# EDM-Research/Real-time-Neural-Rendering-of-LiDAR-Point-Clouds

Hardware: AMD Instinct MI355X
Metric: Mpoints/sec projected + frames/sec at 1920x1080 (higher is better)
Workload: dtype f32

## Files before the change

### real-time-neural-rendering-of-lidar-point-clouds_amd/csrc/rtr_api.hip

```cpp
#include <hip/hip_runtime.h>

#include <algorithm>
#include <cmath>
#include <cstdarg>
#include <cstdio>
#include <cstring>
#include <functional>
#include <string>
#include <vector>

#include "rtr_host.h"
#include "rtr_extract_index.h"

constexpr int kSplitCooldown = 8;

static thread_local std::string g_create_err;

int fail(rtr_ctx *c, int code, const char *fmt, ...) {
    char buf[512];
    va_list ap;
    va_start(ap, fmt);
    vsnprintf(buf, sizeof buf, fmt, ap);
    va_end(ap);
    if (c) c->err = buf; else g_create_err = buf;
// ... 74 lines not shown
    t.cap = 0;
}

int alloc_target(rtr_ctx *c, rtr_ctx::Target &t, int count) {
    free_target(t);
    const size_t npix = (size_t)c->W * c->H, n = (size_t)count * npix;
    const size_t nparts = (size_t)((c->W + 31) / 32) * ((c->H + 31) / 32);
    hipError_t e = rtr::dev_malloc(&t.depth, n * 4);
    if (e == hipSuccess) e = rtr::dev_malloc(&t.img, (n * 3 + 15) & ~(size_t)15);
    if (e == hipSuccess) e = rtr::dev_malloc(&t.tensor, n * 5 * sizeof(uint16_t));
    if (e == hipSuccess) e = rtr::dev_malloc(&t.acc, npix * 16);
    if (e == hipSuccess) e = rtr::dev_malloc(&t.mask, npix);
    if (e == hipSuccess) e = rtr::dev_malloc(&t.part_min, nparts * 4);
    if (e == hipSuccess) e = rtr::dev_malloc(&t.part_max, nparts * 4);
    if (e != hipSuccess) {
        free_target(t);
        return fail(c, RTR_ERR_HIP, "hipMalloc of the frame buffers (%d x %dx%d) failed: %s", count, c->W, c->H,
                    hipGetErrorString(e));
    }
    t.cap = count;
    return RTR_OK;
}

void free_frame(rtr_ctx *c) {
    c->list_valid = false;
    c->split_cooldown = kSplitCooldown;
    free_host_out(c);
    p2p_release(c);
    dfree(c->pp_ids);
    for (auto *t : {&c->frame, &c->views}) {
        free_target(*t);
        for (auto &f : t->fs) {
            dfree(f.store.ext0); dfree(f.store.meta);
            f.nst = f.ntiles = 0;
            f.consts = rtr::StoreConsts{};
        }
    }
    c->W = c->H = 0;
    c->jr.views.count = 0;
}

void reset_pool_sizing(rtr_ctx::Target &t) {
    t.pool_worst = false;
    t.entries_max = 0;
    if (t.entries_host) *t.entries_host = 0u;
}

void free_lists(rtr_ctx *c) {
    if (c->p2p.open || c->p2p.red) p2p_release(c);
    for (auto *t : {&c->frame, &c->views})
        for (auto &f : t->fs) {
            dfree(f.dyn);
            f.dyn_cap = 0;
            f.pool_n = 0;
        }
    c->list_valid = false;
    c->split_cooldown = kSplitCooldown;
    reset_pool_sizing(c->frame);
// ... 180 lines not shown
    rtr_ctx *c; int k; hipStream_t s; hipEvent_t a = nullptr, b = nullptr;
    bool in_dispatch;
    Timed(rtr_ctx *c_, int k_, hipStream_t s_ = nullptr, bool in_dispatch_ = false)
        : c(c_), k(k_), s(s_ ? s_ : c_->stream), in_dispatch(in_dispatch_) {
        if (!c->timing) return;
        if (c->timing >= 2 && k != RTR_K_MIN_DEPTH && k != RTR_K_ACCUMULATE) return;
        if (c->timing == 3 && (c->timing_tick++ & 3u) != 0u) return;
        if (c->timing == 4 && (c->timing_tick++ & 1u) != 0u) return;
        if (c->pool.empty()) {
            (void)hipEventCreate(&a); (void)hipEventCreate(&b);
        } else {
            a = c->pool.back().first; b = c->pool.back().second; c->pool.pop_back();
        }
        if (!in_dispatch) (void)hipEventRecord(a, s);
    }
    ~Timed() {
        if (!a) return;
        if (!in_dispatch) (void)hipEventRecord(b, s);
        c->pending.push_back({a, b, k});
    }
};

hipError_t sync_streams(rtr_ctx *c) {
    if (c->front) {
        hipError_t e = hipStreamSynchronize(c->front);
        if (e != hipSuccess) return e;
    }
    return hipStreamSynchronize(c->stream);
}

#ifndef RTR_DISPATCH_EVENTS
#define RTR_DISPATCH_EVENTS 3
#endif

hipEvent_t consumed_in_dispatch(rtr_ctx *c) {
    if (!(RTR_DISPATCH_EVENTS & 1) || !c->front || !c->frame_overlapped) return nullptr;
    return c->F().consumed;
}

void mark_consumed(rtr_ctx *c, bool in_dispatch = false) {
    if (!c->front || !(c->ov.mode == 1 || c->frame_overlapped)) return;
    auto &f = c->F();
    if (in_dispatch || hipEventRecord(f.consumed, c->stream) == hipSuccess) f.consumed_valid = true;
}

int collect_timing(rtr_ctx *c) {
    if (c->pending.empty()) return RTR_OK;
    HIP_TRY(c, sync_streams(c));
    for (auto &s : c->pending) {
        float ms = 0.f;
        if (hipEventElapsedTime(&ms, s.a, s.b) == hipSuccess) {
            c->total_ms[s.k] += ms;
            c->launches[s.k] += 1;
        }
        c->pool.emplace_back(s.a, s.b);
    }
    c->pending.clear();
    return RTR_OK;
}

int check_frame(rtr_ctx *c) {
    NEED(c, c->W > 0 && c->H > 0, "rtr_set_resolution has not been called");
    return RTR_OK;
}

int check_prefilter(rtr_ctx *c) {
// ... 13 lines not shown
    t.lv_levels = 0;
    for (int i = 1, w = c->W / 2, h = c->H / 2; i <= L; ++i, w /= 2, h /= 2) {
        const hipError_t e = rtr::dev_malloc(&t.lv[i], sizeof(float) * (size_t)w * h);
        if (e != hipSuccess) {
            for (auto &l : t.lv) dfree(l);
            return fail(c, RTR_ERR_HIP, "allocating pyramid level %d (%dx%d) failed: %s", i, w, h, hipGetErrorString(e));
        }
    }
    t.lv_levels = L;
    return RTR_OK;
}

int ensure_pyramid(rtr_ctx *c) {
    if (int rc = check_prefilter(c)) return rc;
    return ensure_levels(c, c->frame);
}

rtr::FilterLevels levels_of(const rtr_ctx *c, const rtr_ctx::Target &t, int k) {
    rtr::FilterLevels L{};
    L.levels = t.lv_levels;
    L.lv[0] = reinterpret_cast<float *>(t.depth + (size_t)k * c->W * c->H);
    L.w[0] = c->W; L.h[0] = c->H;
    for (int i = 1; i <= L.levels; ++i) L.lv[i] = t.lv[i], L.w[i] = L.w[i - 1] / 2, L.h[i] = L.h[i - 1] / 2;
    return L;
}

rtr::TilePyr tile_pyr(const rtr_ctx *c, const rtr_ctx::Target &t, int k, bool enable) {
    rtr::TilePyr pyr{};
    pyr.enable = enable ? 1 : 0;
    if (enable) {
        pyr.L = levels_of(c, t, k);
        pyr.n_eff_rows = (uint32_t)((c->H >> 4) << 4);
        pyr.part_min = t.part_min;
        pyr.part_max = t.part_max;
    }
    return pyr;
}

}

void free_select(rtr_ctx *c) {
    if (!c->sel) return;
    (void)sync_streams(c);
    dfree(c->sel); dfree(c->sel_stats);
}

// ... 116 lines not shown
    if (c->vtab.copied) (void)hipEventDestroy(c->vtab.copied);
    if (c->copy_stream) (void)hipStreamDestroy(c->copy_stream);
    if (c->pp_done) (void)hipEventDestroy(c->pp_done);
    if (c->own_stream) (void)hipStreamDestroy(c->own_stream);
    delete c;
    return RTR_OK;
}

const char *rtr_last_error(const rtr_ctx *c) { return c ? c->err.c_str() : g_create_err.c_str(); }

int rtr_set_params(rtr_ctx *c, const rtr_params *p) {
    if (!c) return RTR_ERR_INVALID;
    c->ov.other_call();
    NEED(c, p != nullptr, "params is NULL");
    NEED(c, p->levels >= 1 && p->levels <= 8, "levels must be in 1..8");
    c->prm = *p;
    c->list_valid = false;
    return RTR_OK;
}

static void overlap_teardown(rtr_ctx *c) {
    if (c->masked_tail && c->stream == c->masked_tail) c->stream = c->own_stream;
    if (c->front) (void)hipStreamDestroy(c->front);
    if (c->masked_tail) (void)hipStreamDestroy(c->masked_tail);
    c->front = c->masked_tail = nullptr;
    for (auto &f : c->frame.fs) {
        if (f.binned) (void)hipEventDestroy(f.binned);
        if (f.consumed) (void)hipEventDestroy(f.consumed);
        f.binned = f.consumed = nullptr;
        f.consumed_valid = false;
    }
    if (c->joined) (void)hipEventDestroy(c->joined);
    c->joined = nullptr;
}

static hipError_t overlap_streams(rtr_ctx *c) {
    if (c->front) return hipSuccess;
    hipError_t e = hipSuccess;
    if (c->ov.mode == 1 && c->opt_tail_cus > 0) {
        uint32_t tail[8] = {0}, head[8] = {0};
        for (int i = 0; i < 256; ++i) {
            int a = i % 8, b = (i / 8) % 4, x = i / 32;
            bool is_tail = b * 8 + (a + x) % 8 < c->opt_tail_cus;
            (is_tail ? tail : head)[i / 32] |= 1u << (i % 32);
        }
        e = hipExtStreamCreateWithCUMask(&c->front, 8, head);
        if (e == hipSuccess) e = hipExtStreamCreateWithCUMask(&c->masked_tail, 8, tail);
        if (e == hipSuccess && c->stream == c->own_stream) c->stream = c->masked_tail;
    } else if (c->opt_front_priority) {
        int least = 0, greatest = 0;
        e = hipDeviceGetStreamPriorityRange(&least, &greatest);
        if (e == hipSuccess) e = hipStreamCreateWithPriority(&c->front, hipStreamNonBlocking, c->opt_front_priority == 1 ? least : greatest);
    } else {
        e = hipStreamCreateWithFlags(&c->front, hipStreamNonBlocking);
    }
    for (int k = 0; k < 2 && e == hipSuccess; ++k) {
        auto &f = c->frame.fs[k];
        e = hipEventCreateWithFlags(&f.binned, hipEventDisableTiming);
        if (e == hipSuccess) e = hipEventCreateWithFlags(&f.consumed, hipEventDisableTiming);
        f.consumed_valid = false;
    }
    if (e == hipSuccess) e = hipEventCreateWithFlags(&c->joined, hipEventDisableTiming);
    if (e != hipSuccess) overlap_teardown(c);
    return e;
}

static int set_overlap(rtr_ctx *c, int value) {
    NEED(c, value >= -1 && value <= 1, "overlap: -1 (automatic), 0 or 1");
    if (value == c->ov.mode && value != 0) return RTR_OK;
    if (value == 1 && c->p2p.open) return fail(c, RTR_ERR_INVALID, "option overlap cannot be switched on while the peer-to-peer exchange is open (rtr_p2p_close first)");
    DevGuard g(c->device);
    HIP_TRY(c, sync_streams(c));
    (void)collect_timing(c);
    if (value == 1 && c->opt_tail_cus > 0) {
        int ncu = 0;
        HIP_TRY(c, hipDeviceGetAttribute(&ncu, hipDeviceAttributeMultiprocessorCount, c->device));
        if (ncu != 256) return fail(c, RTR_ERR_UNSUPPORTED, "tail_cus needs the 256-CU / 8-XCD part (device has %d CUs)", ncu);
    }
    overlap_teardown(c);
    c->ov.set_mode(value);
    if (value == 0) {
        auto &o = c->frame.fs[c->frame.cur ^ 1];
        if (!(c->frame.cur == 1 && (c->p2p.open || c->p2p.red))) {
            dfree(o.dyn); dfree(o.store.ext0); dfree(o.store.meta);
            o.dyn_cap = o.pool_n = 0;
            o.nst = o.ntiles = 0;
            o.consts = rtr::StoreConsts{};
            o.parity = 0;
            o.lean_pending = false;
        }
        return RTR_OK;
    }
    if (value == 1) {
        const hipError_t e = overlap_streams(c);
        if (e != hipSuccess) {
            c->ov.set_mode(0);
            return fail(c, RTR_ERR_HIP, "option overlap: creating the front stream failed: %s", hipGetErrorString(e));
        }
    }
    return RTR_OK;
}

static bool overlap_ready(rtr_ctx *c) {
    if (overlap_streams(c) != hipSuccess) {
        (void)hipGetLastError();
        return false;
    }
    if (c->ov.mode == 1) return true;
    auto &o = c->frame.fs[c->frame.cur ^ 1];
    const std::string err = c->err;
    if (ensure_pool(c, c->frame, o, 0) != RTR_OK || ensure_store(c, c->frame, o, 0, c->front) != RTR_OK) {
        (void)hipGetLastError();
        c->err = err;
        dfree(o.dyn); dfree(o.store.ext0); dfree(o.store.meta);
        o.dyn_cap = o.pool_n = 0;
        o.nst = o.ntiles = 0;
        o.consts = rtr::StoreConsts{};
        return false;
    }
    return true;
}

static int pack_cloud(rtr_ctx *c);

int rtr_set_option(rtr_ctx *c, const char *key, int value) {
    if (!c) return RTR_ERR_INVALID;
    if (key && !strcmp(key, "debug_alloc_fail")) {
        NEED(c, value >= 0, "debug_alloc_fail must be >= 0 (0: off)");
        rtr::alloc_rule().arm(value);
        return RTR_OK;
    }
    c->ov.other_call();
    NEED(c, key != nullptr, "key is NULL");
    if (!strcmp(key, "mode")) {
        NEED(c, value == 0 || value == 1, "mode must be 0 or 1");
        c->opt_mode = value;
        c->list_valid = false;
        return RTR_OK;
    }
    if (!strcmp(key, "point_grid")) {
// ... 178 lines not shown
    else if (!strcmp(key, "nearest_chunks_skipped")) *value = c->nearest_chunks[0];
    else if (!strcmp(key, "nearest_chunks_decoded")) *value = c->nearest_chunks[1];
    else if (!strcmp(key, "nearest_k_given_us")) *value = c->nearest_k_us[0];
    else if (!strcmp(key, "nearest_k_sweep_us")) *value = c->nearest_k_us[1];
    else if (!strcmp(key, "nearest_k_pair_tests_k")) *value = c->nearest_k_tests_k;
    else if (!strcmp(key, "nearest_k_chunks_skipped")) *value = c->nearest_k_chunks[0];
    else if (!strcmp(key, "nearest_k_chunks_decoded")) *value = c->nearest_k_chunks[1];
    else if (!strcmp(key, "nearest_k_cascades_k")) *value = c->nearest_k_cascades_k;
    else if (!strcmp(key, "clusters_keys_us")) *value = c->clusters_us[0];
    else if (!strcmp(key, "clusters_sort_us")) *value = c->clusters_us[1];
    else if (!strcmp(key, "clusters_label_us")) *value = c->clusters_us[2];
    else if (!strcmp(key, "clusters_pair_tests_k")) *value = c->clusters_tests_k;
    else if (!strcmp(key, "plane_sample_us")) *value = c->plane_us[0];
    else if (!strcmp(key, "plane_count_us")) *value = c->plane_us[1];
    else if (!strcmp(key, "point_keep")) *value = c->keep_up ? 1 : 0;
    else if (!strcmp(key, "order_ratio_ppm")) *value = (int)(c->order_ratio * 1e6f);
    else if (!strcmp(key, "cull")) *value = c->opt_cull;
    else if (!strcmp(key, "point_ids")) *value = c->opt_point_ids;
    else if (!strcmp(key, "lane_test")) *value = c->opt_lane_test;
    else if (!strcmp(key, "chunk_test")) *value = c->opt_chunk_test;
    else if (!strcmp(key, "phases")) *value = c->opt_phases;
    else if (!strcmp(key, "overlap")) *value = c->ov.mode;
    else if (!strcmp(key, "overlap_active")) *value = c->ov.active ? 1 : 0;
    else if (!strcmp(key, "front_priority")) *value = c->opt_front_priority;
    else if (!strcmp(key, "lean")) *value = c->opt_lean;
    else if (!strcmp(key, "lean_identity")) *value = c->opt_lean_identity;
    else if (!strcmp(key, "lean_early")) *value = c->opt_lean_early;
    else if (!strcmp(key, "p2p_open")) *value = c->p2p.open ? 1 : 0;
    else if (!strcmp(key, "keep_soa")) *value = c->opt_keep_soa;
    else if (!strcmp(key, "pool_worst_case")) *value = c->opt_pool_worst;
    else if (!strcmp(key, "views")) *value = c->jr.views.count;
    else if (!strcmp(key, "resident_millibytes_per_point")) {
        const uint64_t nchunks = ((c->cap / 4) + 63) / 64;
        uint64_t b = (c->x ? 12 * c->cap : 0) + (c->rgba ? 4 * c->cap : 0) + nchunks * 28 +
                     (c->pk_hdr ? c->pk_bytes + (c->pk_units_cap - c->pk_units) * 32 + 64 : 0) +
                     (c->perm ? 4 * c->cap : 0) + (c->keep_up ? (c->n + 31) / 32 * 4 + nchunks * 33 + 4 : 0) +
                     (c->sel ? std::max<uint64_t>((c->n + 255) / 256, 1) * 32 + 32 : 0);
        const uint64_t npix = (uint64_t)c->W * c->H;
        for (const auto *t : {&c->frame, &c->views}) {
            for (const auto &f : t->fs) {
                b += f.dyn ? f.dyn_cap * 8 : 0;
                b += f.store.ext0 ? ((uint64_t)f.nst * rtr::kS0 + 16) * 8 + rtr::ts_meta_words(f.nst, f.ntiles) * 4 : 0;
            }
            b += t->cap ? npix * (16 + 1 + (uint64_t)t->cap * (4 + 3 + 10)) : 0;
        }
        *value = c->n ? (int)((b * 1000) / c->n > 0x7FFFFFFFull ? 0x7FFFFFFF : (b * 1000) / c->n) : 0;
// ... 1192 lines not shown
    c->W = W; c->H = H;
    if (int rc = alloc_target(c, c->frame, 1)) {
        c->W = c->H = 0;
        return rc;
    }
    return RTR_OK;
}


int rtr_clear(rtr_ctx *c) {
    if (!c) return RTR_ERR_INVALID;
    c->ov.other_call();
    if (int rc = check_frame(c)) return rc;
    DevGuard g(c->device);
    { Timed t(c, RTR_K_CLEAR); rtr::launch_clear(c->stream, c->frame.depth, c->frame.acc, (size_t)c->W * c->H); }
    return launch_check(c, "clear");
}

static bool use_tiles(const rtr_ctx *c) {
    return c->opt_mode == 1 && !c->force_atomic && rtr::tile_count(c->W, c->H) <= 4096;
}

static int bin_points(rtr_ctx *c, const float P[16], bool overlapped, bool clear_split, bool no_split = false,
                      bool lean = false) {
    c->list_valid = false;
    c->last_lean = false;
    c->p2p.occ_current = false;
    c->p2p.occ_from_scan = false;
    hipStream_t s1 = c->stream;
    if (overlapped) {
        if (!c->ov.active) {
            HIP_TRY(c, hipEventRecord(c->joined, c->stream));
            HIP_TRY(c, hipStreamWaitEvent(c->front, c->joined, 0));
        }
        c->frame.cur ^= 1;
        s1 = c->front;
        if (c->F().consumed_valid) HIP_TRY(c, hipStreamWaitEvent(c->front, c->F().consumed, 0));
    }
    if (int rc = ensure_pool(c, c->frame, c->F(), 0)) return rc;
    if (int rc = ensure_store(c, c->frame, c->F(), 0, s1)) return rc;
    auto &t = c->F().store;
    if (c->F().lean_pending && !lean) rtr::launch_lean_fold(s1, c->W, c->H, t, c->F().parity);
    c->F().lean_pending = lean;
    const bool heavy_seen = c->split_cooldown > 0 || __atomic_load_n(c->split_host, __ATOMIC_RELAXED) != 0u;
    t.fill_shift = c->opt_fill_shift >= 0 ? c->opt_fill_shift : (heavy_seen ? 4 : 1);
    if (int rc = next_seq(c, c->F(), s1)) return rc;
    bool binned_in_dispatch = false;
    {
        Timed tm(c, RTR_K_MIN_DEPTH, s1, true);
        binned_in_dispatch = (RTR_DISPATCH_EVENTS & 2) && overlapped && !tm.a && (c->n > 0 || !lean);
        rtr::launch_project_bin(s1, cloud_of(c), make_proj(P), c->W, c->H, t, c->opt_cull ? c->bounds : nullptr,
                                t1_flags(c, clear_split, no_split, lean), c->opt_phases, c->opt_xp, tm.a,
                                binned_in_dispatch ? c->F().binned : tm.b);
        c->p2p.occ_from_scan = c->p2p.open;
    }
    if (overlapped) {
        if (!binned_in_dispatch) HIP_TRY(c, hipEventRecord(c->F().binned, c->front));
        HIP_TRY(c, hipStreamWaitEvent(c->stream, c->F().binned, 0));
    }
    memcpy(c->list_P, P, sizeof c->list_P);
    c->list_valid = true;
    return RTR_OK;
}

int rtr_min_depth_pass(rtr_ctx *c, const float P[16]) {
    if (!c) return RTR_ERR_INVALID;
    c->ov.other_call();
    NEED(c, P != nullptr, "P is NULL");
    if (int rc = check_frame(c)) return rc;
    DevGuard g(c->device);
    c->list_valid = false;
    c->jr.frame.count = 0;
    if (use_tiles(c)) {
        c->frame.pool_worst = true;
        if (int rc = bin_points(c, P, false, c->p2p.whole_frame)) return rc;
        Timed t(c, RTR_K_TILE);
        rtr::launch_tile(c->stream, 1, c->W, c->H, c->F().store, c->prm.depth_window, c->frame.depth, c->frame.acc, c->frame.img,
                         (c->p2p.whole_frame ? 6 : 0) | (c->F().parity << 4), nullptr);
        mark_consumed(c);
// ... 43 lines not shown
int rtr_resolve(rtr_ctx *c) {
    if (!c) return RTR_ERR_INVALID;
    c->ov.other_call();
    if (int rc = check_frame(c)) return rc;
    DevGuard g(c->device);
    { Timed t(c, RTR_K_RESOLVE); rtr::launch_resolve(c->stream, c->frame.acc, c->frame.img, (size_t)c->W * c->H); }
    return launch_check(c, "resolve");
}

int rtr_resolve_range(rtr_ctx *c, const void *acc_dev, uint64_t first_pixel, uint64_t count) {
    if (!c) return RTR_ERR_INVALID;
    c->ov.other_call();
    if (int rc = check_frame(c)) return rc;
    const uint64_t npix = (uint64_t)c->W * c->H;
    NEED(c, first_pixel % 4 == 0 && first_pixel + count <= npix, "bad pixel range (first must be a multiple of 4)");
    if (count == 0) return RTR_OK;
    DevGuard g(c->device);
    const uint32_t *src = acc_dev ? static_cast<const uint32_t *>(acc_dev) : c->frame.acc + first_pixel * 4;
    { Timed t(c, RTR_K_RESOLVE); rtr::launch_resolve(c->stream, src, c->frame.img + first_pixel * 3, (size_t)count); }
    return launch_check(c, "resolve_range");
}

static int filter_impl(rtr_ctx *c, int pyramid_parts, const rtr::Sliced *img_slices = nullptr,
                       const uint32_t *depth_src = nullptr) {
    if (int rc = check_frame(c)) return rc;
    DevGuard g(c->device);
    if (int rc = ensure_pyramid(c)) return rc;
    {
        Timed t(c, RTR_K_FILTER);
        rtr::launch_filter(c->stream, levels_of(c, c->frame, 0), c->frame.depth, c->frame.img, c->frame.mask, c->frame.tensor, c->frame.minmax, c->frame.part_min, c->frame.part_max,
                           c->W, c->H, c->prm.filter_strength, c->prm.gradient_threshold, pyramid_parts, img_slices,
                           depth_src);
    }
    return launch_check(c, "filter");
}

int rtr_filter(rtr_ctx *c) {
    if (!c) return RTR_ERR_INVALID;
    c->ov.other_call();
    return filter_impl(c, 0);
}


int rtr_render(rtr_ctx *c, const float P[16], int with_filter) {
    if (!c) return RTR_ERR_INVALID;
    NEED(c, P != nullptr, "P is NULL");
    if (int rc = check_frame(c)) return rc;
    c->jr.pass.behind = false;
    if (with_filter) {
        DevGuard g(c->device);
        if (int rc = ensure_pyramid(c)) return rc;
    }
    int rc;
    bool fused = false;
    if (use_tiles(c)) {
        DevGuard g(c->device);
        bool overlapped = c->ov.frame(!c->p2p.open && (c->ov.mode == 1 || !c->p2p.red), with_filter != 0, c->W, c->H, c->cloud_seq);
        if (overlapped && !c->ov.active && !overlap_ready(c)) {
            c->ov.resources_failed();
            overlapped = false;
        }
        c->frame_overlapped = overlapped;
        bool split_launch = c->opt_heavy > 0;
        if (split_launch) {
            if (__atomic_load_n(c->split_host, __ATOMIC_RELAXED) != 0u) c->split_cooldown = kSplitCooldown;
            split_launch = c->split_cooldown > 0;
            if (c->split_cooldown > 0) --c->split_cooldown;
        }
        const bool lean = c->opt_lean && !split_launch && !c->p2p.open;
        if ((rc = bin_points(c, P, overlapped, !overlapped, !split_launch, lean))) {
            c->frame_overlapped = false;
            c->ov.other_call();
            return rc;
        }
        if (lean) {
            c->F().parity ^= 1;
            c->last_lean = true;
        }
        if (overlapped && split_launch) rtr::launch_reset_split(c->stream, c->W, c->H, c->F().store, c->frame.depth, c->frame.acc);
        fused = with_filter && c->prm.levels == 4;
        const rtr::TilePyr pyr = tile_pyr(c, c->frame, 0, fused);
        const hipEvent_t consumed = consumed_in_dispatch(c);
        {
            Timed t(c, RTR_K_TILE);
            rtr::launch_tile(c->stream, 0, c->W, c->H, c->F().store, c->prm.depth_window, c->frame.depth, c->frame.acc, c->frame.img,
                             c->opt_keep_accum | (lean ? lean_bits(c, c->frame) : 0) | (c->F().parity << 4), fused ? &pyr : nullptr,
                             nullptr, split_launch ? nullptr : consumed);
            if (lean) c->list_valid = false;
            if (split_launch)
                rtr::launch_tile(c->stream, 3, c->W, c->H, c->F().store, c->prm.depth_window, c->frame.depth, c->frame.acc, c->frame.img,
                                 c->opt_keep_accum, fused ? &pyr : nullptr, nullptr, consumed);
        }
        mark_consumed(c, consumed != nullptr);
        c->frame_overlapped = false;
        c->ov.frame_done(overlapped);
        if ((rc = launch_check(c, "tile frame"))) return rc;
        auto &rec = c->jr.frame;
        memcpy(rec.P, P, sizeof(float) * 16);
        rec.filter = with_filter;
        rec.count = 1;
        rec.clip = c->clip;
    } else {
        (void)c->ov.frame(false, false, c->W, c->H, c->cloud_seq);
        c->ov.frame_done(false);
        c->force_atomic = true;
        rc = rtr_clear(c);
        if (!rc) rc = rtr_min_depth_pass(c, P);
        if (!rc) rc = rtr_accumulate_pass(c, P);
        if (!rc) rc = rtr_resolve(c);
        c->force_atomic = false;
        if (rc) return rc;
    }
    if (with_filter) return filter_impl(c, fused ? rtr::tile_count(c->W, c->H) : 0);
    return RTR_OK;
}

static int frame_to_host(rtr_ctx *c, const float P[16], uint8_t *host_img, float *host_depth, int with_filter) {
    if (!c) return RTR_ERR_INVALID;
    if (!host_img && !host_depth) return fail(c, RTR_ERR_NO_OUTPUT, "both outputs are NULL (project_cloud.cu:270-273)");
    c->ov.other_call();
    if (int rc = rtr_render(c, P, with_filter)) return rc;
    DevGuard g(c->device);
    const size_t npix = (size_t)c->W * c->H;
    const Copy copies[2] = {{host_depth, c->frame.depth, npix * 4}, {host_img, c->frame.img, npix * 3}};
    HIP_TRY(c, queue_copies(c, copies, 2));
    HIP_TRY(c, sync_streams(c));
    rtr_ctx::Journal::Frames own;
    memcpy(own.P, P, sizeof(float) * 16);
    own.count = 1;
    own.filter = with_filter;
    own.clip = c->clip;
    return repair(c, c->frame, false, copies, 2, &own);
}

int rtr_project(rtr_ctx *c, const float P[16], uint8_t *host_img, float *host_depth) {
    return frame_to_host(c, P, host_img, host_depth, 0);
// ... 654 lines not shown
```

### real-time-neural-rendering-of-lidar-point-clouds_amd/csrc/rtr_host.h

```cpp
#pragma once
#include <hip/hip_runtime.h>

#include <string>
#include <utility>
#include <vector>

#include "../../include/rtr.h"
#include "rtr_alloc.h"
#include "rtr_kernels.h"
#include "rtr_overlap_policy.h"

struct rtr_ctx {
    int device = 0;
    hipStream_t own_stream = nullptr;
    hipStream_t stream = nullptr;
    rtr_params prm{};
    std::string err;

    float *x = nullptr, *y = nullptr, *z = nullptr;
    uint32_t *rgba = nullptr;
    float *bounds = nullptr;
    float *spread = nullptr;
    float absmax[3] = {0.f, 0.f, 0.f};
    int opt_lane_test = 1;
// ... 4 lines not shown
    int opt_lean_identity = 1;
    int opt_lean_early = -1;
    bool last_lean = false;
    uint64_t n = 0, cap = 0;
    uint4 *pk_hdr = nullptr;
    uint32_t *pk_planes = nullptr, *pk_planes_b = nullptr;
    uint64_t pk_bytes = 0;
    uint64_t pk_units = 0, pk_units_cap = 0;
    uint64_t pk_hdr_chunks = 0;
    int opt_pack = 1;

    int W = 0, H = 0;
    rtr::Clip clip{};

    struct FrontSet {
        rtr::TileStore store{};
        uint64_t pool_n = 0;
        int nst = 0, ntiles = 0;
        rtr::StoreConsts consts{};
        uint64_t *dyn = nullptr;
        uint64_t dyn_cap = 0;
        hipEvent_t binned = nullptr, consumed = nullptr;
        bool consumed_valid = false;
        int parity = 0;
        bool lean_pending = false;
    };

    struct Target {
        int cap = 0;
        uint32_t *depth = nullptr, *acc = nullptr, *part_min = nullptr, *part_max = nullptr;
        uint8_t *img = nullptr, *mask = nullptr;
        uint16_t *tensor = nullptr;
        uint32_t *minmax = nullptr;
        float *lv[9] = {nullptr};
        int lv_levels = 0;
        FrontSet fs[RTR_MAX_VIEWS];
        int cur = 0;
        uint32_t *err_host = nullptr, *err_dev = nullptr;
        uint32_t *entries_host = nullptr, *entries_dev = nullptr;
        uint64_t entries_max = 0;
        bool pool_worst = false;
    } frame, views;
    FrontSet &F() { return frame.fs[frame.cur]; }
    rtr::OverlapPolicy ov;
    bool frame_overlapped = false;
    int opt_front_priority = 0;
    int opt_tail_cus = 0;
    hipStream_t front = nullptr;
    hipStream_t masked_tail = nullptr;
    hipEvent_t joined = nullptr;
    bool list_valid = false;
    float list_P[12] = {0};
    int opt_mode = 1;
    int opt_keep_accum = 0;
    bool force_atomic = false;
    int opt_heavy = 32768;
    int opt_slice = 16384;
    int opt_p2p_timeout_ms = 2000;
    int opt_fill_shift = -1;
    int opt_debug_dyn_cap = -1;
    int opt_debug_extract_window = -1;
    uint32_t debug_store_stamp = 0;
    int opt_debug_p2p_barrier = -1;
    uint32_t *split_host = nullptr, *split_dev = nullptr;
    int split_cooldown = 0;
    int opt_xp = 0;
    int opt_phases = 0;
    int opt_probe = 0;
    int opt_cull = 0;
    int opt_auto_reorder = 2;
    bool reordered = false;
// ... 172 lines not shown
```

### real-time-neural-rendering-of-lidar-point-clouds_amd/csrc/rtr_kernels.h

```cpp
#pragma once
#include <hip/hip_runtime.h>
#include <stdint.h>

#include "rtr_barrier_rule.h"
#include "rtr_chunk_box.h"
#include "rtr_stamp_rule.h"

namespace rtr {

struct Proj {
    float m[12];
};

constexpr uint32_t kPackMaxBits = 25;
struct PackedXyz {
    const uint4 *hdr;
    const uint32_t *planes;
    const uint32_t *planes_b;
};
constexpr uint64_t pack_b_dwords(uint64_t units) { return (units * 2 + 256 + 16 + 15) & ~15ull; }
constexpr uint64_t pack_total_dwords(uint64_t units) { return pack_b_dwords(units) + units * 6 + 16; }

struct Cloud {
    const float *x, *y, *z;
// ... 138 lines not shown
size_t view_tab_bytes();
hipError_t launch_project_bin_views(hipStream_t s, const Cloud &c, const Proj *P, const TileStore *S, int count, int W, int H,
                              void *tab_host, void *tab_dev, int flags, int phases, hipEvent_t ev_start = nullptr,
                              hipEvent_t ev_stop = nullptr);
void launch_chunk_bounds(hipStream_t s, const Cloud &c, float *bounds, float *spread);
void pack_measure(hipStream_t s, const Cloud &c, uint4 *hdr, uint32_t *chunk_planes, uint64_t *total_planes,
                  uint64_t first_unit = 0);
void pack_write(hipStream_t s, const Cloud &c, const uint4 *hdr, uint32_t *planes, uint32_t *planes_b);
void pack_verify(hipStream_t s, const Cloud &c, const uint4 *hdr, const uint32_t *planes, const uint32_t *planes_b, uint64_t *mismatches);
void unpack_to_soa(hipStream_t s, const PackedXyz &pk, uint64_t n, float *x, float *y, float *z);
int reorder_morton(hipStream_t s, float *x, float *y, float *z, uint32_t *rgba, uint64_t n, uint32_t *perm = nullptr);
size_t order_quality_scratch_bytes();
int order_quality(hipStream_t s, const float *bounds, uint64_t n, float *ratio, float absmax[3], void *scratch = nullptr);
void launch_reset_split(hipStream_t s, int W, int H, const TileStore &S, uint32_t *depth, uint32_t *acc);
void launch_tile(hipStream_t s, int mode, int W, int H, const TileStore &S, float window, uint32_t *depth,
                 uint32_t *acc, uint8_t *img, int write_acc, const TilePyr *pyr, const Sliced *depth_slices = nullptr,
                 hipEvent_t ev_stop = nullptr);
void launch_lean_fold(hipStream_t s, int W, int H, const TileStore &S, int parity);
void launch_stream_probe(hipStream_t s, const Cloud &c, const Proj &P, int W, int H, uint32_t *sink, int variant);
void launch_resolve(hipStream_t s, const uint32_t *acc, uint8_t *img, size_t npix);
void launch_filter(hipStream_t s, const FilterLevels &L, uint32_t *depth_bits, uint8_t *img, uint8_t *mask,
                   uint16_t *tensor, uint32_t *minmax, uint32_t *part_min, uint32_t *part_max, int W, int H,
                   float strength, float thr, int pyramid_parts, const Sliced *img_slices = nullptr,
                   const uint32_t *depth_src = nullptr);
void launch_p2p_sync(hipStream_t s, uint32_t *my_flags, const PeerSet &peer_flags, int rank, int world, uint32_t seq,
                     uint32_t *status, unsigned long long timeout_ticks);
void launch_p2p_sync_gather(hipStream_t s, uint32_t *my_flags, const PeerSet &peer_flags, int rank, int world, uint32_t seq,
                            uint32_t *status, unsigned long long timeout_ticks, const PeerSet &occ, uint32_t *occ_all);
constexpr int kP2POccBytes = 512;
void launch_p2p_collect(hipStream_t s, int W, int H, const OwnedTab *tab, const uint32_t *occ_all, int world, int rank,
                        uint32_t *depth, uint8_t *img, const TilePyr *pyr);
void launch_p2p_occupancy(hipStream_t s, const uint32_t *tile_cnt, int W, int H, uint32_t *occ);
void launch_p2p_depth_reduce(hipStream_t s, const PeerSet &depth, const PeerSet &occ, uint32_t *red, size_t first,
                             size_t count, int world, int W, int H);
void launch_p2p_gather(hipStream_t s, const PeerSet &src, void *dst, size_t chunk_bytes, size_t nbytes,
                       int skip_owner);
void launch_p2p_acc_resolve(hipStream_t s, const PeerSet &acc, const PeerSet &occ, uint8_t *img, size_t first,
                            size_t count, int world, int W, int H);
void launch_generate(hipStream_t s, int scene, uint64_t seed, uint64_t first, uint64_t count, uint64_t total,
                     float *x, float *y, float *z, uint32_t *rgba);
void launch_aos_to_soa(hipStream_t s, const uint8_t *xyz, size_t xyz_stride, const uint8_t *rgb, size_t rgb_stride,
                       uint64_t count, float *x, float *y, float *z, uint32_t *rgba);
void launch_soa_to_aos(hipStream_t s, const float *x, const float *y, const float *z, const uint32_t *rgba,
                       uint64_t count, float *xyzw, uint8_t *rgba_out);
void launch_copy_to_host(hipStream_t s, const void *a, void *ha, size_t bytes_a, const void *b, void *hb, size_t bytes_b);
void launch_pad_nan(hipStream_t s, float *x, float *y, float *z, uint32_t *rgba, uint64_t n, uint64_t n_pad);
void launch_point_pass(hipStream_t s, const Cloud &c, const Proj &P, int W, int H, const uint32_t *depth, float window,
// ... 108 lines not shown
```

### real-time-neural-rendering-of-lidar-point-clouds_amd/csrc/rtr_kernels.hip

```cpp
#include "rtr_device.h"
#include "rtr_lane_test.h"
#include "rtr_remove_index.h"
#include "rtr_extract_index.h"

#include <hip/hip_ext.h>
#include <hip/hip_fp16.h>

#include <type_traits>

namespace rtr {

__global__ __launch_bounds__(kBlock) void k_clear(uint4 *__restrict__ depth4, uint4 *__restrict__ acc4,
                                                  size_t n_depth4, size_t n_acc4, uint32_t *depth, size_t npix) {
    size_t i = (size_t)blockIdx.x * kBlock + threadIdx.x;
    size_t stride = (size_t)gridDim.x * kBlock;
    const uint4 e = make_uint4(RTR_EMPTY, RTR_EMPTY, RTR_EMPTY, RTR_EMPTY);
    const uint4 z = make_uint4(0, 0, 0, 0);
    for (size_t j = i; j < n_acc4; j += stride) acc4[j] = z;
    for (size_t j = i; j < n_depth4; j += stride) depth4[j] = e;
    for (size_t j = n_depth4 * 4 + i; j < npix; j += stride) depth[j] = RTR_EMPTY;
}

void launch_clear(hipStream_t s, uint32_t *depth, uint32_t *acc, size_t npix) {
    size_t n_acc4 = npix, n_depth4 = npix / 4;
// ... 3017 lines not shown
        const int gx = ox + q % SX, gy = oy + q / SX;
        if (gx < 0 || gx >= hw || gy < 0 || gy >= hh) continue;
        if (!keep_px(lo, hi[q], gx, gy, strength, thr)) hi[q] = bilerp(lo, gx, gy);
    }
}

#ifdef RTR_EXPERIMENT
__device__ unsigned long long g_fstamp[2][8];
#define RTR_FSTAMP(k) do { if (threadIdx.x == 0 && (blockIdx.x == 5 || blockIdx.x == 1900)) g_fstamp[blockIdx.x == 5 ? 0 : 1][k] = wall_clock64(); } while (0)
void read_filter_stamps(hipStream_t s, unsigned long long *out16) {
    (void)hipMemcpyFromSymbolAsync(out16, HIP_SYMBOL(g_fstamp), sizeof g_fstamp, 0, hipMemcpyDeviceToHost, s);
}
#else
#define RTR_FSTAMP(k) do { } while (0)
#endif
__global__ __launch_bounds__(kBlock) void k_filter4(const float *__restrict__ g1, const float *__restrict__ g2,
                                                    const float *__restrict__ g3, const float *__restrict__ g4,
                                                    int h4, float *__restrict__ depth, uint8_t *__restrict__ img,
                                                    uint8_t *__restrict__ mask, uint16_t *__restrict__ tensor,
                                                    const uint32_t *__restrict__ part_min,
                                                    const uint32_t *__restrict__ part_max, int nparts,
                                                    uint32_t *__restrict__ minmax, int W, int H, int blocks_x,
                                                    float strength, float thr, Sliced isl,
                                                    const float *__restrict__ depth_src) {
    __shared__ float s1[kF1x * kF1y], s2[kF2x * kF2y], s3[kF3x * kF3y], s4[kF4x * kF4y];
    __shared__ uint32_t s_mm[8];
    __shared__ uint16_t s_lut[256];
    static_assert(kBlock == 256, "one table entry per thread");
    RTR_FSTAMP(0);
    s_lut[threadIdx.x] = (uint16_t)colour_half(threadIdx.x);
    const int X0 = (blockIdx.x % blocks_x) * kFuseW, Y0 = (blockIdx.x / blocks_x) * kFuseH;
    const int t = threadIdx.x, x = X0 + 4 * (t & 15), y = Y0 + (t >> 4);
    const bool inb = x < W && y < H;
    const size_t npix = (size_t)W * H, idx = (size_t)y * W + x;
    float4 d4 = make_float4(0.f, 0.f, 0.f, 0.f);
    uint32_t iw0 = 0, iw1 = 0, iw2 = 0;
    if (inb) {
        d4 = *reinterpret_cast<const float4 *>(depth_src + idx);
        const uint8_t *src = isl.chunk ? static_cast<const uint8_t *>(isl.src.p[idx / isl.chunk]) : img;
        const uint32_t *ip = reinterpret_cast<const uint32_t *>(src + idx * 3);
        iw0 = ip[0]; iw1 = ip[1]; iw2 = ip[2];
    }
    const int w1 = W >> 1, w2 = W >> 2, w3 = W >> 3, w4 = W >> 4, h3 = 2 * h4, h2 = 4 * h4, h1 = 8 * h4;
    const int x1 = (X0 >> 1) - 1, y1 = (Y0 >> 1) - 1, x2 = (X0 >> 2) - 2, y2 = (Y0 >> 2) - 2;
    const int x3 = (X0 >> 3) - 2, y3 = (Y0 >> 3) - 2, x4 = (X0 >> 4) - 2, y4 = (Y0 >> 4) - 2;
    stage_level<kF1x, kF1y>(s1, x1, y1, g1, w1, h1);
    stage_level<kF2x, kF2y>(s2, x2, y2, g2, w2, h2);
    stage_level<kF3x, kF3y>(s3, x3, y3, g3, w3, h3);
    stage_level<kF4x, kF4y>(s4, x4, y4, g4, w4, h4);
    RTR_FSTAMP(1);
    uint32_t fa = 0xFFFFFFFFu, fb = 0u;
    {
        const int n4p = nparts >> 2;
        const uint4 *const pm4 = reinterpret_cast<const uint4 *>(part_min), *const px4 = reinterpret_cast<const uint4 *>(part_max);
        for (int k = t; k < n4p; k += kBlock) {
            const uint4 a = pm4[k], b = px4[k];
            const uint32_t a2 = a.x < a.y ? a.x : a.y, a3 = a.z < a.w ? a.z : a.w, b2 = b.x > b.y ? b.x : b.y, b3 = b.z > b.w ? b.z : b.w;
            const uint32_t pa = a2 < a3 ? a2 : a3, pb = b2 > b3 ? b2 : b3;
            fa = pa < fa ? pa : fa;
            fb = pb > fb ? pb : fb;
        }
        for (int k = 4 * n4p + t; k < nparts; k += kBlock) {
// ... 19 lines not shown
    up_level<kF2x, kF2y>(s2, x2, y2, w2, h2, LdsLevel{s3, x3, y3, kF3x, w3, h3}, strength, thr);
    __syncthreads();
    up_level<kF1x, kF1y>(s1, x1, y1, w1, h1, LdsLevel{s2, x2, y2, kF2x, w2, h2}, strength, thr);
    __syncthreads();
    RTR_FSTAMP(3);
#pragma unroll
    for (int k = 0; k < 4; ++k) {
        fa = s_mm[k] < fa ? s_mm[k] : fa;
        fb = s_mm[4 + k] > fb ? s_mm[4 + k] : fb;
    }
    if (blockIdx.x == 0 && t == 0) {
        minmax[0] = fa;
        minmax[1] = fb;
    }
    const float mn = __uint_as_float(fa), range = f_sub(__uint_as_float(fb), mn);
    if (!inb) return;
    final_quad(LdsLevel{s1, x1, y1, kF1x, w1, h1}, d4, iw0, iw1, iw2, depth, img, mask, tensor, mn, range,
               x, y, idx, npix, y < 2 * h1, strength, thr, s_lut);
    RTR_FSTAMP(4);
}

void launch_filter(hipStream_t s, const FilterLevels &L, uint32_t *depth_bits, uint8_t *img, uint8_t *mask,
                   uint16_t *tensor, uint32_t *minmax, uint32_t *part_min, uint32_t *part_max, int W, int H,
                   float strength, float thr, int pyramid_parts, const Sliced *img_slices, const uint32_t *depth_src) {
    auto blocks = [](size_t n) { return dim3((unsigned)((n + kBlock - 1) / kBlock)); };
    const int nl = L.levels;
    const int h_eff = (H >> nl) << nl;
    const int tiles_x = (W + 31) / 32, tiles_y = (H + 31) / 32;
    int nparts = tiles_x * tiles_y;
    if (nl == 4) {
        if (pyramid_parts == 0)
            hipLaunchKernelGGL(k_pyramid, dim3(nparts), dim3(kBlock), 0, s, L, tiles_x, (uint32_t)h_eff, part_min, part_max);
        const int bx = (W + kFuseW - 1) / kFuseW, by = (H + kFuseH - 1) / kFuseH;
        hipLaunchKernelGGL(k_filter4, dim3(bx * by), dim3(kBlock), 0, s, L.lv[1], L.lv[2], L.lv[3], L.lv[4], L.h[4],
                           (float *)depth_bits, img, mask, tensor, part_min, part_max,
                           pyramid_parts > 0 ? pyramid_parts : nparts, minmax, W, H, bx, strength, thr,
                           img_slices ? *img_slices : Sliced{}, (const float *)(depth_src ? depth_src : depth_bits));
        return;
    }
    {
        FilterLevels L4 = L;
        if (L4.levels > 4) L4.levels = 4;
        hipLaunchKernelGGL(k_pyramid, dim3(nparts), dim3(kBlock), 0, s, L4, tiles_x, (uint32_t)h_eff, part_min, part_max);
    }
    for (int i = 5; i <= nl; ++i)
        hipLaunchKernelGGL(k_reduce, blocks((size_t)L.w[i] * L.h[i]), dim3(kBlock), 0, s, L.lv[i - 1], L.lv[i], L.w[i],
                           L.h[i]);
    int cw = L.w[nl], ch = L.h[nl];
    bool first = true;
    for (int i = nl; i >= 2; --i) {
        hipLaunchKernelGGL(k_up, blocks((size_t)4 * cw * ch), dim3(kBlock), 0, s, L.lv[i], L.lv[i - 1], cw, ch, strength,
                           thr, first ? part_min : nullptr, first ? part_max : nullptr, nparts, minmax);
        first = false;
        cw *= 2;
        ch *= 2;
    }
    if (first) {
        hipLaunchKernelGGL(k_up, dim3(1), dim3(kBlock), 0, s, L.lv[1], L.lv[0], 0, 0, strength, thr, part_min, part_max,
                           nparts, minmax);
    }
// ... 811 lines not shown
```

Baseline: 1.069 million.

## Run projection and tiling on alternating lane streams with per-set staging buffers

Adds a second front stream and per-frame-set staging buffers (depth, image, pyramid levels, part min/max) so projection, binning and the fused tile/pyramid pass of one frame write into private buffers on their own lane. The filter on the main stream reads from those buffers, with consumed/filtered events ordering reuse. The aim is to let frame N+1's front-end work overlap frame N's filter without waiting on the shared frame buffers. In exchange it costs extra device memory and more event synchronisation, and it only applies when overlap is active with levels==4, filtering on, and no split launch.

```diff
diff --git a/real-time-neural-rendering-of-lidar-point-clouds_amd/csrc/rtr_api.hip b/real-time-neural-rendering-of-lidar-point-clouds_amd/csrc/rtr_api.hip
--- a/real-time-neural-rendering-of-lidar-point-clouds_amd/csrc/rtr_api.hip
+++ b/real-time-neural-rendering-of-lidar-point-clouds_amd/csrc/rtr_api.hip
@@ -120,6 +120,32 @@
     return RTR_OK;
 }
 
+void free_lane_bufs(rtr_ctx::FrontSet &f) {
+    dfree(f.pre_depth); dfree(f.pre_img); dfree(f.pre_min); dfree(f.pre_max);
+    for (auto &l : f.pre_lv) dfree(l);
+    f.pre_w = f.pre_h = 0;
+}
+
+hipError_t ensure_lane_bufs(rtr_ctx *c, rtr_ctx::FrontSet &f) {
+    if (f.pre_depth && f.pre_w == c->W && f.pre_h == c->H) return hipSuccess;
+    free_lane_bufs(f);
+    const size_t npix = (size_t)c->W * c->H;
+    const size_t nparts = (size_t)((c->W + 31) / 32) * ((c->H + 31) / 32);
+    hipError_t e = rtr::dev_malloc(&f.pre_depth, npix * 4);
+    if (e == hipSuccess) e = rtr::dev_malloc(&f.pre_img, (npix * 3 + 15) & ~(size_t)15);
+    if (e == hipSuccess) e = rtr::dev_malloc(&f.pre_min, nparts * 4);
+    if (e == hipSuccess) e = rtr::dev_malloc(&f.pre_max, nparts * 4);
+    for (int i = 1, w = c->W / 2, h = c->H / 2; i <= 4 && e == hipSuccess; ++i, w /= 2, h /= 2)
+        e = rtr::dev_malloc(&f.pre_lv[i], sizeof(float) * (size_t)w * h);
+    if (e != hipSuccess) {
+        free_lane_bufs(f);
+        return e;
+    }
+    f.pre_w = c->W;
+    f.pre_h = c->H;
+    return hipSuccess;
+}
+
 void free_frame(rtr_ctx *c) {
     c->list_valid = false;
     c->split_cooldown = kSplitCooldown;
@@ -132,6 +158,7 @@
             dfree(f.store.ext0); dfree(f.store.meta);
             f.nst = f.ntiles = 0;
             f.consts = rtr::StoreConsts{};
+            free_lane_bufs(f);
         }
     }
     c->W = c->H = 0;
@@ -358,8 +385,9 @@
 };
 
 hipError_t sync_streams(rtr_ctx *c) {
-    if (c->front) {
-        hipError_t e = hipStreamSynchronize(c->front);
+    for (hipStream_t s : {c->front, c->lane1}) {
+        if (!s) continue;
+        hipError_t e = hipStreamSynchronize(s);
         if (e != hipSuccess) return e;
     }
     return hipStreamSynchronize(c->stream);
@@ -374,10 +402,11 @@
     return c->F().consumed;
 }
 
-void mark_consumed(rtr_ctx *c, bool in_dispatch = false) {
+void mark_consumed(rtr_ctx *c, bool in_dispatch = false, hipStream_t on = nullptr) {
     if (!c->front || !(c->ov.mode == 1 || c->frame_overlapped)) return;
     auto &f = c->F();
-    if (in_dispatch || hipEventRecord(f.consumed, c->stream) == hipSuccess) f.consumed_valid = true;
+    if (!on) on = c->stream;
+    if (in_dispatch || hipEventRecord(f.consumed, on) == hipSuccess) f.consumed_valid = true, f.reader = on;
 }
 
 int collect_timing(rtr_ctx *c) {
@@ -437,6 +466,15 @@
     L.lv[0] = reinterpret_cast<float *>(t.depth + (size_t)k * c->W * c->H);
     L.w[0] = c->W; L.h[0] = c->H;
     for (int i = 1; i <= L.levels; ++i) L.lv[i] = t.lv[i], L.w[i] = L.w[i - 1] / 2, L.h[i] = L.h[i - 1] / 2;
+    return L;
+}
+
+rtr::FilterLevels lane_levels(const rtr_ctx *c, const rtr_ctx::FrontSet &f) {
+    rtr::FilterLevels L{};
+    L.levels = 4;
+    L.lv[0] = reinterpret_cast<float *>(f.pre_depth);
+    L.w[0] = c->W; L.h[0] = c->H;
+    for (int i = 1; i <= 4; ++i) L.lv[i] = f.pre_lv[i], L.w[i] = L.w[i - 1] / 2, L.h[i] = L.h[i - 1] / 2;
     return L;
 }
 
@@ -599,13 +637,16 @@
 static void overlap_teardown(rtr_ctx *c) {
     if (c->masked_tail && c->stream == c->masked_tail) c->stream = c->own_stream;
     if (c->front) (void)hipStreamDestroy(c->front);
+    if (c->lane1) (void)hipStreamDestroy(c->lane1);
     if (c->masked_tail) (void)hipStreamDestroy(c->masked_tail);
-    c->front = c->masked_tail = nullptr;
+    c->front = c->lane1 = c->masked_tail = nullptr;
     for (auto &f : c->frame.fs) {
         if (f.binned) (void)hipEventDestroy(f.binned);
         if (f.consumed) (void)hipEventDestroy(f.consumed);
-        f.binned = f.consumed = nullptr;
-        f.consumed_valid = false;
+        if (f.filtered) (void)hipEventDestroy(f.filtered);
+        f.binned = f.consumed = f.filtered = nullptr;
+        f.consumed_valid = f.filtered_valid = false;
+        f.reader = nullptr;
     }
     if (c->joined) (void)hipEventDestroy(c->joined);
     c->joined = nullptr;
@@ -628,14 +669,18 @@
         int least = 0, greatest = 0;
         e = hipDeviceGetStreamPriorityRange(&least, &greatest);
         if (e == hipSuccess) e = hipStreamCreateWithPriority(&c->front, hipStreamNonBlocking, c->opt_front_priority == 1 ? least : greatest);
+        if (e == hipSuccess) e = hipStreamCreateWithPriority(&c->lane1, hipStreamNonBlocking, c->opt_front_priority == 1 ? least : greatest);
     } else {
         e = hipStreamCreateWithFlags(&c->front, hipStreamNonBlocking);
+        if (e == hipSuccess) e = hipStreamCreateWithFlags(&c->lane1, hipStreamNonBlocking);
     }
     for (int k = 0; k < 2 && e == hipSuccess; ++k) {
         auto &f = c->frame.fs[k];
         e = hipEventCreateWithFlags(&f.binned, hipEventDisableTiming);
         if (e == hipSuccess) e = hipEventCreateWithFlags(&f.consumed, hipEventDisableTiming);
-        f.consumed_valid = false;
+        if (e == hipSuccess) e = hipEventCreateWithFlags(&f.filtered, hipEventDisableTiming);
+        f.consumed_valid = f.filtered_valid = false;
+        f.reader = nullptr;
     }
     if (e == hipSuccess) e = hipEventCreateWithFlags(&c->joined, hipEventDisableTiming);
     if (e != hipSuccess) overlap_teardown(c);
@@ -657,6 +702,7 @@
     overlap_teardown(c);
     c->ov.set_mode(value);
     if (value == 0) {
+        for (int k = 0; k < 2; ++k) free_lane_bufs(c->frame.fs[k]);
         auto &o = c->frame.fs[c->frame.cur ^ 1];
         if (!(c->frame.cur == 1 && (c->p2p.open || c->p2p.red))) {
             dfree(o.dyn); dfree(o.store.ext0); dfree(o.store.meta);
@@ -686,13 +732,17 @@
     if (c->ov.mode == 1) return true;
     auto &o = c->frame.fs[c->frame.cur ^ 1];
     const std::string err = c->err;
-    if (ensure_pool(c, c->frame, o, 0) != RTR_OK || ensure_store(c, c->frame, o, 0, c->front) != RTR_OK) {
+    bool ok = ensure_pool(c, c->frame, o, 0) == RTR_OK && ensure_store(c, c->frame, o, 0, c->front) == RTR_OK;
+    if (c->lane1 && c->prm.levels == 4)
+        for (int k = 0; k < 2 && ok; ++k) ok = ensure_lane_bufs(c, c->frame.fs[k]) == hipSuccess;
+    if (!ok) {
         (void)hipGetLastError();
         c->err = err;
         dfree(o.dyn); dfree(o.store.ext0); dfree(o.store.meta);
         o.dyn_cap = o.pool_n = 0;
         o.nst = o.ntiles = 0;
         o.consts = rtr::StoreConsts{};
+        for (int k = 0; k < 2; ++k) free_lane_bufs(c->frame.fs[k]);
         return false;
     }
     return true;
@@ -917,6 +967,7 @@
     else if (!strcmp(key, "phases")) *value = c->opt_phases;
     else if (!strcmp(key, "overlap")) *value = c->ov.mode;
     else if (!strcmp(key, "overlap_active")) *value = c->ov.active ? 1 : 0;
+    else if (!strcmp(key, "overlap_lanes")) *value = c->ov.active && c->last_lane ? 1 : 0;
     else if (!strcmp(key, "front_priority")) *value = c->opt_front_priority;
     else if (!strcmp(key, "lean")) *value = c->opt_lean;
     else if (!strcmp(key, "lean_identity")) *value = c->opt_lean_identity;
@@ -2155,7 +2206,7 @@
 }
 
 static int bin_points(rtr_ctx *c, const float P[16], bool overlapped, bool clear_split, bool no_split = false,
-                      bool lean = false) {
+                      bool lean = false, bool lane = false) {
     c->list_valid = false;
     c->last_lean = false;
     c->p2p.occ_current = false;
@@ -2165,10 +2216,12 @@
         if (!c->ov.active) {
             HIP_TRY(c, hipEventRecord(c->joined, c->stream));
             HIP_TRY(c, hipStreamWaitEvent(c->front, c->joined, 0));
+            if (c->lane1) HIP_TRY(c, hipStreamWaitEvent(c->lane1, c->joined, 0));
         }
         c->frame.cur ^= 1;
-        s1 = c->front;
-        if (c->F().consumed_valid) HIP_TRY(c, hipStreamWaitEvent(c->front, c->F().consumed, 0));
+        s1 = lane ? c->lane(c->frame.cur) : c->front;
+        auto &f = c->F();
+        if (f.consumed_valid && f.reader != s1) HIP_TRY(c, hipStreamWaitEvent(s1, f.consumed, 0));
     }
     if (int rc = ensure_pool(c, c->frame, c->F(), 0)) return rc;
     if (int rc = ensure_store(c, c->frame, c->F(), 0, s1)) return rc;
@@ -2181,13 +2234,13 @@
     bool binned_in_dispatch = false;
     {
         Timed tm(c, RTR_K_MIN_DEPTH, s1, true);
-        binned_in_dispatch = (RTR_DISPATCH_EVENTS & 2) && overlapped && !tm.a && (c->n > 0 || !lean);
+        binned_in_dispatch = (RTR_DISPATCH_EVENTS & 2) && overlapped && !lane && !tm.a && (c->n > 0 || !lean);
         rtr::launch_project_bin(s1, cloud_of(c), make_proj(P), c->W, c->H, t, c->opt_cull ? c->bounds : nullptr,
                                 t1_flags(c, clear_split, no_split, lean), c->opt_phases, c->opt_xp, tm.a,
                                 binned_in_dispatch ? c->F().binned : tm.b);
         c->p2p.occ_from_scan = c->p2p.open;
     }
-    if (overlapped) {
+    if (overlapped && !lane) {
         if (!binned_in_dispatch) HIP_TRY(c, hipEventRecord(c->F().binned, c->front));
         HIP_TRY(c, hipStreamWaitEvent(c->stream, c->F().binned, 0));
     }
@@ -2277,15 +2330,20 @@
 }
 
 static int filter_impl(rtr_ctx *c, int pyramid_parts, const rtr::Sliced *img_slices = nullptr,
-                       const uint32_t *depth_src = nullptr) {
+                       const uint32_t *depth_src = nullptr, const rtr_ctx::FrontSet *lane_set = nullptr) {
     if (int rc = check_frame(c)) return rc;
     DevGuard g(c->device);
     if (int rc = ensure_pyramid(c)) return rc;
     {
         Timed t(c, RTR_K_FILTER);
-        rtr::launch_filter(c->stream, levels_of(c, c->frame, 0), c->frame.depth, c->frame.img, c->frame.mask, c->frame.tensor, c->frame.minmax, c->frame.part_min, c->frame.part_max,
-                           c->W, c->H, c->prm.filter_strength, c->prm.gradient_threshold, pyramid_parts, img_slices,
-                           depth_src);
+        if (lane_set)
+            rtr::launch_filter(c->stream, lane_levels(c, *lane_set), c->frame.depth, c->frame.img, c->frame.mask, c->frame.tensor, c->frame.minmax, lane_set->pre_min, lane_set->pre_max,
+                               c->W, c->H, c->prm.filter_strength, c->prm.gradient_threshold, pyramid_parts, nullptr,
+                               lane_set->pre_depth, lane_set->pre_img);
+        else
+            rtr::launch_filter(c->stream, levels_of(c, c->frame, 0), c->frame.depth, c->frame.img, c->frame.mask, c->frame.tensor, c->frame.minmax, c->frame.part_min, c->frame.part_max,
+                               c->W, c->H, c->prm.filter_strength, c->prm.gradient_threshold, pyramid_parts, img_slices,
+                               depth_src);
     }
     return launch_check(c, "filter");
 }
@@ -2308,6 +2366,7 @@
     }
     int rc;
     bool fused = false;
+    rtr_ctx::FrontSet *lane_set = nullptr;
     if (use_tiles(c)) {
         DevGuard g(c->device);
         bool overlapped = c->ov.frame(!c->p2p.open && (c->ov.mode == 1 || !c->p2p.red), with_filter != 0, c->W, c->H, c->cloud_seq);
@@ -2323,7 +2382,18 @@
             if (c->split_cooldown > 0) --c->split_cooldown;
         }
         const bool lean = c->opt_lean && !split_launch && !c->p2p.open;
-        if ((rc = bin_points(c, P, overlapped, !overlapped, !split_launch, lean))) {
+        bool lane = overlapped && c->lane1 && with_filter && c->prm.levels == 4 && !split_launch && !c->opt_keep_accum;
+        if (lane && ensure_lane_bufs(c, c->frame.fs[c->frame.cur ^ 1]) != hipSuccess) {
+            const hipError_t e = hipGetLastError();
+            if (c->ov.mode == 1) {
+                c->frame_overlapped = false;
+                c->ov.other_call();
+                return fail(c, RTR_ERR_HIP, "allocating the lane buffers of an overlapped frame failed: %s", hipGetErrorString(e));
+            }
+            lane = false;
+        }
+        c->last_lane = lane;
+        if ((rc = bin_points(c, P, overlapped, !overlapped, !split_launch, lean, lane))) {
             c->frame_overlapped = false;
             c->ov.other_call();
             return rc;
@@ -2334,11 +2404,19 @@
         }
         if (overlapped && split_launch) rtr::launch_reset_split(c->stream, c->W, c->H, c->F().store, c->frame.depth, c->frame.acc);
         fused = with_filter && c->prm.levels == 4;
-        const rtr::TilePyr pyr = tile_pyr(c, c->frame, 0, fused);
-        const hipEvent_t consumed = consumed_in_dispatch(c);
+        rtr::TilePyr pyr = tile_pyr(c, c->frame, 0, fused);
+        if (lane) {
+            pyr.L = lane_levels(c, c->F());
+            pyr.part_min = c->F().pre_min;
+            pyr.part_max = c->F().pre_max;
+        }
+        const hipEvent_t consumed = lane ? c->F().consumed : consumed_in_dispatch(c);
+        const hipStream_t ts = lane ? c->lane(c->frame.cur) : c->stream;
+        if (lane && c->F().filtered_valid) HIP_TRY(c, hipStreamWaitEvent(ts, c->F().filtered, 0));
         {
-            Timed t(c, RTR_K_TILE);
-            rtr::launch_tile(c->stream, 0, c->W, c->H, c->F().store, c->prm.depth_window, c->frame.depth, c->frame.acc, c->frame.img,
+            Timed t(c, RTR_K_TILE, ts);
+            rtr::launch_tile(ts, 0, c->W, c->H, c->F().store, c->prm.depth_window, lane ? c->F().pre_depth : c->frame.depth, c->frame.acc,
+                             lane ? c->F().pre_img : c->frame.img,
                              c->opt_keep_accum | (lean ? lean_bits(c, c->frame) : 0) | (c->F().parity << 4), fused ? &pyr : nullptr,
                              nullptr, split_launch ? nullptr : consumed);
             if (lean) c->list_valid = false;
@@ -2346,10 +2424,14 @@
                 rtr::launch_tile(c->stream, 3, c->W, c->H, c->F().store, c->prm.depth_window, c->frame.depth, c->frame.acc, c->frame.img,
                                  c->opt_keep_accum, fused ? &pyr : nullptr, nullptr, consumed);
         }
-        mark_consumed(c, consumed != nullptr);
+        mark_consumed(c, consumed != nullptr, ts);
         c->frame_overlapped = false;
         c->ov.frame_done(overlapped);
         if ((rc = launch_check(c, "tile frame"))) return rc;
+        if (lane) {
+            HIP_TRY(c, hipStreamWaitEvent(c->stream, c->F().consumed, 0));
+            lane_set = &c->F();
+        }
         auto &rec = c->jr.frame;
         memcpy(rec.P, P, sizeof(float) * 16);
         rec.filter = with_filter;
@@ -2366,7 +2448,12 @@
         c->force_atomic = false;
         if (rc) return rc;
     }
-    if (with_filter) return filter_impl(c, fused ? rtr::tile_count(c->W, c->H) : 0);
+    if (!with_filter) return RTR_OK;
+    if ((rc = filter_impl(c, fused ? rtr::tile_count(c->W, c->H) : 0, nullptr, nullptr, lane_set))) return rc;
+    if (lane_set) {
+        HIP_TRY(c, hipEventRecord(lane_set->filtered, c->stream));
+        lane_set->filtered_valid = true;
+    }
     return RTR_OK;
 }
 
diff --git a/real-time-neural-rendering-of-lidar-point-clouds_amd/csrc/rtr_host.h b/real-time-neural-rendering-of-lidar-point-clouds_amd/csrc/rtr_host.h
--- a/real-time-neural-rendering-of-lidar-point-clouds_amd/csrc/rtr_host.h
+++ b/real-time-neural-rendering-of-lidar-point-clouds_amd/csrc/rtr_host.h
@@ -50,6 +50,13 @@
         uint64_t dyn_cap = 0;
         hipEvent_t binned = nullptr, consumed = nullptr;
         bool consumed_valid = false;
+        hipStream_t reader = nullptr;
+        uint32_t *pre_depth = nullptr, *pre_min = nullptr, *pre_max = nullptr;
+        uint8_t *pre_img = nullptr;
+        float *pre_lv[5] = {nullptr};
+        int pre_w = 0, pre_h = 0;
+        hipEvent_t filtered = nullptr;
+        bool filtered_valid = false;
         int parity = 0;
         bool lean_pending = false;
     };
@@ -72,9 +79,12 @@
     FrontSet &F() { return frame.fs[frame.cur]; }
     rtr::OverlapPolicy ov;
     bool frame_overlapped = false;
+    bool last_lane = false;
     int opt_front_priority = 0;
     int opt_tail_cus = 0;
     hipStream_t front = nullptr;
+    hipStream_t lane1 = nullptr;
+    hipStream_t lane(int set) const { return set ? lane1 : front; }
     hipStream_t masked_tail = nullptr;
     hipEvent_t joined = nullptr;
     bool list_valid = false;
diff --git a/real-time-neural-rendering-of-lidar-point-clouds_amd/csrc/rtr_kernels.h b/real-time-neural-rendering-of-lidar-point-clouds_amd/csrc/rtr_kernels.h
--- a/real-time-neural-rendering-of-lidar-point-clouds_amd/csrc/rtr_kernels.h
+++ b/real-time-neural-rendering-of-lidar-point-clouds_amd/csrc/rtr_kernels.h
@@ -184,7 +184,7 @@
 void launch_filter(hipStream_t s, const FilterLevels &L, uint32_t *depth_bits, uint8_t *img, uint8_t *mask,
                    uint16_t *tensor, uint32_t *minmax, uint32_t *part_min, uint32_t *part_max, int W, int H,
                    float strength, float thr, int pyramid_parts, const Sliced *img_slices = nullptr,
-                   const uint32_t *depth_src = nullptr);
+                   const uint32_t *depth_src = nullptr, const uint8_t *img_src = nullptr);
 void launch_p2p_sync(hipStream_t s, uint32_t *my_flags, const PeerSet &peer_flags, int rank, int world, uint32_t seq,
                      uint32_t *status, unsigned long long timeout_ticks);
 void launch_p2p_sync_gather(hipStream_t s, uint32_t *my_flags, const PeerSet &peer_flags, int rank, int world, uint32_t seq,
diff --git a/real-time-neural-rendering-of-lidar-point-clouds_amd/csrc/rtr_kernels.hip b/real-time-neural-rendering-of-lidar-point-clouds_amd/csrc/rtr_kernels.hip
--- a/real-time-neural-rendering-of-lidar-point-clouds_amd/csrc/rtr_kernels.hip
+++ b/real-time-neural-rendering-of-lidar-point-clouds_amd/csrc/rtr_kernels.hip
@@ -3063,7 +3063,8 @@
                                                     const uint32_t *__restrict__ part_max, int nparts,
                                                     uint32_t *__restrict__ minmax, int W, int H, int blocks_x,
                                                     float strength, float thr, Sliced isl,
-                                                    const float *__restrict__ depth_src) {
+                                                    const float *__restrict__ depth_src,
+                                                    const uint8_t *__restrict__ img_src) {
     __shared__ float s1[kF1x * kF1y], s2[kF2x * kF2y], s3[kF3x * kF3y], s4[kF4x * kF4y];
     __shared__ uint32_t s_mm[8];
     __shared__ uint16_t s_lut[256];
@@ -3078,7 +3079,7 @@
     uint32_t iw0 = 0, iw1 = 0, iw2 = 0;
     if (inb) {
         d4 = *reinterpret_cast<const float4 *>(depth_src + idx);
-        const uint8_t *src = isl.chunk ? static_cast<const uint8_t *>(isl.src.p[idx / isl.chunk]) : img;
+        const uint8_t *src = isl.chunk ? static_cast<const uint8_t *>(isl.src.p[idx / isl.chunk]) : img_src;
         const uint32_t *ip = reinterpret_cast<const uint32_t *>(src + idx * 3);
         iw0 = ip[0]; iw1 = ip[1]; iw2 = ip[2];
     }
@@ -3144,7 +3145,8 @@
 
 void launch_filter(hipStream_t s, const FilterLevels &L, uint32_t *depth_bits, uint8_t *img, uint8_t *mask,
                    uint16_t *tensor, uint32_t *minmax, uint32_t *part_min, uint32_t *part_max, int W, int H,
-                   float strength, float thr, int pyramid_parts, const Sliced *img_slices, const uint32_t *depth_src) {
+                   float strength, float thr, int pyramid_parts, const Sliced *img_slices, const uint32_t *depth_src,
+                   const uint8_t *img_src) {
     auto blocks = [](size_t n) { return dim3((unsigned)((n + kBlock - 1) / kBlock)); };
     const int nl = L.levels;
     const int h_eff = (H >> nl) << nl;
@@ -3157,7 +3159,8 @@
         hipLaunchKernelGGL(k_filter4, dim3(bx * by), dim3(kBlock), 0, s, L.lv[1], L.lv[2], L.lv[3], L.lv[4], L.h[4],
                            (float *)depth_bits, img, mask, tensor, part_min, part_max,
                            pyramid_parts > 0 ? pyramid_parts : nparts, minmax, W, H, bx, strength, thr,
-                           img_slices ? *img_slices : Sliced{}, (const float *)(depth_src ? depth_src : depth_bits));
+                           img_slices ? *img_slices : Sliced{}, (const float *)(depth_src ? depth_src : depth_bits),
+                           (const uint8_t *)(img_src ? img_src : img));
         return;
     }
     {
```

Result: slower. 283,600 (-73.5%).
